# 14chanwa/remotesensingProject

Measured on AMD Instinct MI355X. Metric: Mpixel*disparity-hypotheses/s, higher is better.
Workload: dtype f32

## Files before the change

### remotesensingproject_amd/csrc/k2_reg.hpp

```cpp
#pragma once

#include "k2_scan.hpp"

namespace rslf {

#ifndef RSLF_REG_GB104
#define RSLF_REG_GB104 8
#endif
constexpr int gather_batch(int c) { return c == 1 ? 8 : 4; }
constexpr int kPadSlack = 16;

template <int SPAD, int C, bool PK, bool KONLY>
__device__ __forceinline__ void mean_shift_pass(const float (&R)[PK ? 1 : C][PK ? 1 : SPAD], const f2 (&R2)[PK ? C : 1][PK ? SPAD / 2 : 1],
                                                int S, float kq, const float (&rbar)[C], float (&A)[C], float& B)
{
    static_assert(!KONLY || (C == 1 && !PK), "the K-only pass is written for the scalar one-channel blocks");
    if constexpr (PK) {
        f2 rb2[C];
        const f2 kq2 = {kq, kq};
#pragma unroll
        for (int c = 0; c < C; c++)
            rb2[c] = f2{rbar[c], rbar[c]};
        constexpr int kBlk = (C == 1) ? 8 : 4;
#pragma unroll
        for (int s0 = 0; s0 < SPAD; s0 += kBlk) {
            if (!(s0 < SPAD - kPadSlack || s0 < S))
                continue;
            if constexpr (C == 1) {
                f2 P[4], K[4];
                const f2 r4[4] = {R2[0][s0 / 2], R2[0][s0 / 2 + 1], R2[0][s0 / 2 + 2], R2[0][s0 / 2 + 3]};
                mean_shift_pk_octet(r4, rb2[0], kq2, P, K);
#pragma unroll
                for (int j = 0; j < 4; j++) {
                    A[0] = A[0] + P[j].x;
                    B = B + K[j].x;
                    A[0] = A[0] + P[j].y;
                    B = B + K[j].y;
                }
            } else {
                f2 Pa[3], Pb[3], Ka, Kb;
                const f2 ra[3] = {R2[0][s0 / 2], R2[1][s0 / 2], R2[C - 1][s0 / 2]};
                const f2 rb[3] = {R2[0][s0 / 2 + 1], R2[1][s0 / 2 + 1], R2[C - 1][s0 / 2 + 1]};
                const f2 m[3] = {rb2[0], rb2[C > 1 ? 1 : 0], rb2[C - 1]};
                mean_shift_pk_rgb_quad(ra, rb, m, kq2, Pa, Pb, Ka, Kb);
#pragma unroll
                for (int c = 0; c < C; c++)
                    A[c] = A[c] + Pa[c].x;
                B = B + Ka.x;
#pragma unroll
                for (int c = 0; c < C; c++)
                    A[c] = A[c] + Pa[c].y;
                B = B + Ka.y;
#pragma unroll
                for (int c = 0; c < C; c++)
                    A[c] = A[c] + Pb[c].x;
                B = B + Kb.x;
#pragma unroll
                for (int c = 0; c < C; c++)
                    A[c] = A[c] + Pb[c].y;
                B = B + Kb.y;
            }
        }
    } else if (C == 1) {
#pragma unroll
        for (int s0 = 0; s0 < SPAD; s0 += 4) {
            if (s0 + 4 <= SPAD - kPadSlack || s0 + 4 <= S) {
                if constexpr (KONLY)
                    mean_shift_group4_k(R[0][s0], R[0][s0 + 1], R[0][s0 + 2], R[0][s0 + 3], rbar[0], kq, B);
                else
                    mean_shift_group4(R[0][s0], R[0][s0 + 1], R[0][s0 + 2], R[0][s0 + 3], rbar[0], kq, A[0], B);
            } else {
#pragma unroll
                for (int j = 0; j < 3; j++)
                    if (s0 + j < S) {
                        if constexpr (KONLY)
                            mean_shift_group1_k(R[0][s0 + j], rbar[0], kq, B);
                        else
                            mean_shift_group1(R[0][s0 + j], rbar[0], kq, A[0], B);
                    }
            }
        }
    } else {
#pragma unroll
        for (int s = 0; s < SPAD; s++) {
            if (!(s < SPAD - kPadSlack || s < S))
                continue;
            float q[C];
#pragma unroll
            for (int c = 0; c < C; c++) {
                const float delta = R[c][s] - rbar[c];
                const float tq = kq * delta;
                q[c] = tq * delta;
            }
            float qs = q[0];
            if (C == 3) {
                qs = q[0] + q[C - 1];
                qs = qs + q[C > 1 ? 1 : 0];
            }
            const float K = kernel_weight(qs);
#pragma unroll
            for (int c = 0; c < C; c++) {
                const float pr = R[c][s] * K;
                A[c] = A[c] + pr;
            }
            B = B + K;
        }
    }
}

template <int SPAD, int C, bool BORDER, bool UNIFORM_D, bool PK, int GB = 0, class BestT = Best<C>, bool LANE_D = false,
          bool TRIM = false>
__device__ __forceinline__ void scan_reg_body(const ScanArgs& a, int v, int u, int d0, int d1, BestT& best,
                                              float* __restrict__ otab, int dlane = 0, int dstep = 1)
{
    static_assert(!LANE_D || !UNIFORM_D, "hypotheses in the lanes: every lane has its own view offsets");
    constexpr int kGatherBatch = GB > 0 ? GB : (C == 1 && !PK && SPAD == 104 && RSLF_REG_GB104 == 13) ? 13 : gather_batch(C);
    static_assert(SPAD % kGatherBatch == 0 && (!PK || kGatherBatch % 2 == 0), "whole batches, whole pairs");
    static_assert(SPAD % 8 == 0, "slot counts are multiples of 8");
    const VolView& vol = a.vol;
    const float* epi = vol.row(v, 0);
    const float uf = (float)u;
    const int Um1 = vol.U - 1;
    const unsigned Um1_bits = __float_as_uint((float)Um1);
    const int S = vol.S;
    const int lane = threadIdx.x & 63;
    const long long o = (long long)v * vol.U + u;
    const float dmin = a.dmin_vu ? a.dmin_vu[o] : a.dmin;
    const float dmax = a.dmax_vu ? a.dmax_vu[o] : a.dmax;
    const float range = dmax - dmin;
    const float denom = (float)(a.dim_d - 1);
    const float kq = (C == 1) ? a.k.k1 : a.k.inv_h2;
    const float slope = a.k.slope;
    const int stride_s = (int)vol.stride_s;
    float centre[C];
#pragma unroll
    for (int c = 0; c < C; c++)
        centre[c] = epi[(long long)a.s_hat * vol.stride_s + u * C + c];

#pragma unroll 1
    for (int dk = d0; dk < d1; dk += (LANE_D ? dstep : 1)) {
        const int d = LANE_D ? min(dk + dlane, d1 - 1) : dk;
        const float Dd = hypothesis(dmin, range, denom, d);
        float R[PK ? 1 : C][PK ? 1 : SPAD];
        f2 R2[PK ? C : 1][PK ? SPAD / 2 : 1];
        int card = BORDER ? 0 : S;
        float Ss0 = (float)a.s_hat;
        asm volatile("" : "+v"(Ss0));
        int rowoff = 0;
        asm volatile("" : "+s"(rowoff));
        if (UNIFORM_D) {
#pragma unroll
            for (int s0 = 0; s0 < SPAD; s0 += 64) {
                const int s = s0 + lane;
                float off = (float)(a.s_hat - s) * Dd;
                off = off * slope;
                if (SPAD % 64 == 0 || s < SPAD)
                    otab[s] = off;
            }
            __builtin_amdgcn_wave_barrier();
        }
#pragma unroll
        for (int g = 0; g < SPAD / kGatherBatch; g++) {
            float tt[kGatherBatch], e0[C][kGatherBatch], e1[C][kGatherBatch];
            bool ok[kGatherBatch];
#pragma unroll
            for (int j = 0; j < kGatherBatch; j++) {
                const int s = g * kGatherBatch + j;
                tt[j] = 0.0f;
                ok[j] = false;
#pragma unroll
                for (int c = 0; c < C; c++) {
                    e0[c][j] = kSentinel;
                    e1[c][j] = 0.0f;
                }
                if (s < SPAD - kPadSlack || s < S) {
                    float x;
                    if (UNIFORM_D) {
                        x = otab[s];
                    } else {
                        x = (Ss0 - (float)s) * Dd;
                        x = x * slope;
                    }
                    x = x + uf;
                    tt[j] = lerp_weight(x);
                    int i0 = floor_to_int(x);
                    ok[j] = true;
                    if (BORDER) {
                        ok[j] = __float_as_uint(x) <= Um1_bits;
                        i0 = ok[j] ? i0 : 0;
                    }
                    const unsigned byteoff = (unsigned)(i0 * C + rowoff) << 2;
                    const float* p = (const float*)((const char*)epi + byteoff);
#pragma unroll
                    for (int c = 0; c < C; c++) {
                        e0[c][j] = p[c];
                        e1[c][j] = p[C + c];
                    }
                }
                rowoff += stride_s;
            }
#pragma unroll
            for (int j = 0; j < kGatherBatch; j++) {
                const int s = g * kGatherBatch + j;
                const float omt = 1.0f - tt[j];
#pragma unroll
                for (int c = 0; c < C; c++) {
                    const float m0 = omt * e0[c][j];
                    const float m1 = tt[j] * e1[c][j];
                    const float r = m0 + m1;
                    float val;
                    if (BORDER)
                        val = ok[j] ? r : kSentinel;
                    else
                        val = (s < SPAD - kPadSlack || s < S) ? r : kSentinel;
                    if constexpr (PK) {
                        if (s & 1)
                            R2[c][s >> 1].y = val;
                        else
                            R2[c][s >> 1].x = val;
                    } else {
                        R[c][s] = val;
                    }
                }
                if (BORDER)
                    card += ok[j] ? 1 : 0;
            }
            {
                const int b = g * kGatherBatch;
#pragma unroll
                for (int c = 0; c < C; c++) {
                    if constexpr (PK) {
                        asm volatile("" : "+v"(R2[c][b / 2]), "+v"(R2[c][b / 2 + 1]));
                        if (kGatherBatch == 8)
                            asm volatile("" : "+v"(R2[c][b / 2 + 2]), "+v"(R2[c][b / 2 + 3]));
                        static_assert(!PK || kGatherBatch == 4 || kGatherBatch == 8, "pair pinning is written for 4 and 8");
                    } else if (kGatherBatch != 4 && kGatherBatch != 8) {
#pragma unroll
                        for (int j = 0; j < kGatherBatch; j++)
                            asm volatile("" : "+v"(R[c][b + j]));
                    } else {
                        asm volatile("" : "+v"(R[c][b + 0]), "+v"(R[c][b + 1]), "+v"(R[c][b + 2]), "+v"(R[c][b + 3]));
                        if (kGatherBatch == 8)
                            asm volatile("" : "+v"(R[c][b + kGatherBatch - 4]), "+v"(R[c][b + kGatherBatch - 3]),
                                              "+v"(R[c][b + kGatherBatch - 2]), "+v"(R[c][b + kGatherBatch - 1]));
                    }
                }
                if (BORDER)
                    asm volatile("" : "+s"(rowoff), "+v"(Ss0), "+v"(card));
                else
                    asm volatile("" : "+s"(rowoff), "+v"(Ss0));
            }
        }

        float rbar[C];
#pragma unroll
        for (int c = 0; c < C; c++)
            rbar[c] = centre[c];
        float B = 0.0f;
#pragma unroll 1
        for (int it = 0; it < a.k.n_iter; it++) {
            float A[C];
#pragma unroll
            for (int c = 0; c < C; c++)
                A[c] = 0.0f;
            B = 0.0f;
            if constexpr (TRIM) {
                if (it == a.k.n_iter - 1) {
                    mean_shift_pass<SPAD, C, PK, true>(R, R2, S, kq, rbar, A, B);
                    break;
                }
            }
            mean_shift_pass<SPAD, C, PK, false>(R, R2, S, kq, rbar, A, B);
#pragma unroll
            for (int c = 0; c < C; c++) {
                const float qd = (B != 0.0f) ? (A[c] / B) : 0.0f;
                rbar[c] = (qd > 0.0f) ? qd : 0.0f;
            }
        }
        const float cardf = (float)card;
        float sc = (card != 0) ? (B / cardf) : 0.0f;
        sc = (sc > 0.0f) ? sc : 0.0f;
        if (!LANE_D || dk + dlane < d1)
            best.offer(sc, d, Dd, rbar);
    }
}

template <int C>
struct LastPassRbar {
    __device__ __forceinline__ void operator()(const ScanArgs& a, long long o, float Dd, float (&rbar)[C]) const
    {
        if (a.k.n_iter == 0)
            return;
        const VolView& vol = a.vol;
        const int v = (int)(o / vol.U);
        const int u = (int)(o - (long long)v * vol.U);
        const float* epi = vol.row(v, 0);
        const float uf = (float)u;
        const unsigned Um1_bits = __float_as_uint((float)(vol.U - 1));
        const float kq = (C == 1) ? a.k.k1 : a.k.inv_h2;
        const float Ss0 = (float)a.s_hat;
        const int S = vol.S;
        float A[C];
#pragma unroll
        for (int c = 0; c < C; c++)
            A[c] = 0.0f;
        float B = 0.0f;
        constexpr int kBatch = 8;
#pragma unroll 1
        for (int s0 = 0; s0 < S; s0 += kBatch) {
            float R[C][kBatch];
#pragma unroll
            for (int j = 0; j < kBatch; j++) {
                const int s = min(s0 + j, S - 1);
                float x = (Ss0 - (float)s) * Dd;
                x = x * a.k.slope;
                x = x + uf;
                const float t = lerp_weight(x);
                const bool ok = __float_as_uint(x) <= Um1_bits;
                const int i0 = ok ? floor_to_int(x) : 0;
                const float* p = epi + (long long)s * vol.stride_s + i0 * C;
                const float omt = 1.0f - t;
#pragma unroll
                for (int c = 0; c < C; c++) {
                    const float m0 = omt * p[c];
                    const float m1 = t * p[C + c];
                    const float r = m0 + m1;
                    R[c][j] = ok ? r : kSentinel;
                }
            }
#pragma unroll
            for (int j = 0; j < kBatch; j++) {
                if (s0 + j >= S)
                    break;
                float q[C];
#pragma unroll
                for (int c = 0; c < C; c++) {
                    const float delta = R[c][j] - rbar[c];
                    const float tq = kq * delta;
                    q[c] = tq * delta;
                }
                float qs = q[0];
                if (C == 3) {
                    qs = q[0] + q[C - 1];
                    qs = qs + q[C > 1 ? 1 : 0];
                }
                const float K = kernel_weight(qs);
#pragma unroll
                for (int c = 0; c < C; c++) {
                    const float pr = R[c][j] * K;
                    A[c] = A[c] + pr;
                }
                B = B + K;
            }
        }
#pragma unroll
        for (int c = 0; c < C; c++) {
            const float qd = (B != 0.0f) ? (A[c] / B) : 0.0f;
            rbar[c] = (qd > 0.0f) ? qd : 0.0f;
        }
    }
};

constexpr int scan_reg_waves(int spad, int c)
{
    const int regs = ((c * spad + (c == 1 ? 64 : 96) + 7) / 8) * 8;
    const int w = 512 / regs;
    if (c == 1 && spad > 104 && spad <= 144) return 3;
    if (c == 1 && spad >= 80 && spad <= 88) return 4;
    if (c == 3 && spad >= 32 && spad <= 40) return 3;
    if (c == 1 && (spad == 48 || spad == 40)) return 5;
    if (c == 3 && spad == 24) return 4;
    if (c == 1 && spad == 16) return 7;
    return w > 8 ? 8 : (w < 1 ? 1 : w);
}

#ifndef RSLF_REG_BEST_LDS
#define RSLF_REG_BEST_LDS 1
#endif
constexpr bool scan_reg_best_in_lds(int spad, int c)
{
    if (!RSLF_REG_BEST_LDS)
        return false;
    if (c == 1)
        return spad == 16 || spad == 40 || spad == 48 || (spad >= 80 && spad <= 88) || (spad >= 104 && spad <= 144);
    return spad == 24 || spad == 40;
}

constexpr bool scan_reg_packed_math(int spad, int c) { return scan_reg_waves(spad, c) == 1; }

constexpr bool scan_reg_trim(int spad, int c)
{
    return c == 1 && !scan_reg_packed_math(spad, c) && spad != 48 && !(spad >= 80 && spad <= 88) && !(spad > 112 && spad <= 144);
}
template <int SPAD, int C>
using ScanRegRbarFix = std::conditional_t<scan_reg_trim(SPAD, C), LastPassRbar<C>, NoRbarFix>;

template <int SPAD, int C, class BestT>
__device__ __forceinline__ void scan_reg_rows(const ScanArgs& a, int v, int u, int d0, int d1, BestT& best, float* otab)
{
    constexpr bool PK = scan_reg_packed_math(SPAD, C);
    if (a.dmin_vu) {
        scan_reg_body<SPAD, C, true, false, PK, 0, BestT, false, scan_reg_trim(SPAD, C)>(a, v, u, d0, d1, best, otab);
        return;
    }
    const float max_ds = (float)max(a.s_hat, a.vol.S - 1 - a.s_hat);
    const float range = a.dmax - a.dmin, denom = (float)(a.dim_d - 1);
    const float uf = (float)u, Um1 = (float)(a.vol.U - 1);
    auto interior = [&](int d) -> bool {
        const float reach = max_ds * fabsf(hypothesis(a.dmin, range, denom, d)) * fabsf(a.k.slope) + 2.0f;
        return __all((uf - reach >= 0.0f) && (uf + reach <= Um1));
    };
    int d = d0;
    while (d < d1) {
        const bool in = interior(d);
        int e = d + 1;
        while (e < d1 && interior(e) == in)
            e++;
        if (in)
            scan_reg_body<SPAD, C, false, true, PK, 0, BestT, false, scan_reg_trim(SPAD, C)>(a, v, u, d, e, best, otab);
        else
            scan_reg_body<SPAD, C, true, true, PK, 0, BestT, false, scan_reg_trim(SPAD, C)>(a, v, u, d, e, best, otab);
        d = e;
    }
}

template <int SPAD, int C>
__global__ __launch_bounds__(64 * kScanWaves) __attribute__((amdgpu_waves_per_eu(scan_reg_waves(SPAD, C), scan_reg_waves(SPAD, C))))
void k2_scan_reg(ScanArgs a)
{
    __shared__ float s_otab[kScanWaves][SPAD];
    float* otab = s_otab[__builtin_amdgcn_readfirstlane(threadIdx.x >> 6)];
    constexpr bool kEpiDyn = false;
    float* const epi_lds = nullptr;
    const int epi_stride = 0;
    using Fix = ScanRegRbarFix<SPAD, C>;
    if constexpr (scan_reg_best_in_lds(SPAD, C)) {
        __shared__ float s_best[kScanWaves][BestLds<C>::kFloats];
        BestLds<C> running(s_best[__builtin_amdgcn_readfirstlane(threadIdx.x >> 6)]);
        RSLF_SCAN_ROW_TILE_FIX((running.init(), scan_reg_rows<SPAD, C>(a, v, u, d0, d1, running, otab), running.load(best)), Fix{})
    } else {
        RSLF_SCAN_ROW_TILE_FIX((scan_reg_rows<SPAD, C>(a, v, u, d0, d1, best, otab)), Fix{})
    }
}

#ifndef RSLF_PACKED_LONG_GB
#define RSLF_PACKED_LONG_GB 4
#endif
constexpr bool packed_long_unit(int spad, int c) { return c == 1 && spad >= 80 && spad <= 128 && spad % RSLF_PACKED_LONG_GB == 0; }
constexpr int packed_waves(int spad, int c) { return packed_long_unit(spad, c) ? 2 : scan_reg_waves(spad + 24, c); }
constexpr int packed_gather_batch(int spad, int c) { return packed_long_unit(spad, c) ? spad / RSLF_PACKED_LONG_GB : 0; }

template <int SPAD, int C>
__global__ __launch_bounds__(64 * kScanWaves) __attribute__((amdgpu_waves_per_eu(packed_waves(SPAD, C), packed_waves(SPAD, C))))
void k2_scan_reg_packed(ScanArgs a)
{
    constexpr bool kEpiDyn = false;
    float* const epi_lds = nullptr;
    const int epi_stride = 0;
    RSLF_SCAN_PACKED_LOOP((scan_reg_body<SPAD, C, true, false, packed_waves(SPAD, C) == 1, packed_gather_batch(SPAD, C)>(a, v, u, d0, d1, best, nullptr)))
}

#ifndef RSLF_PX_ROWLIKE
#define RSLF_PX_ROWLIKE 1
#endif
constexpr int px_kernel_waves(int spad, int c) { return RSLF_PX_ROWLIKE ? scan_reg_waves(spad, c) : packed_waves(spad, c); }
template <int SPAD, int C>
__global__ __launch_bounds__(64 * kScanWaves) __attribute__((amdgpu_waves_per_eu(px_kernel_waves(SPAD, C), px_kernel_waves(SPAD, C))))
void k2_scan_reg_px(ScanArgs a)
{
    __shared__ double s_sum[kScanWaves];
    __shared__ float s_rec[kScanWaves][kPxRecFloats];
    const int n = *a.packed_n;
    const int lane = threadIdx.x & 63;
    const int wave = __builtin_amdgcn_readfirstlane(threadIdx.x >> 6);
    const int wpp = a.px_waves, ppw = kScanWaves / wpp;
    const int items = (n + ppw - 1) / ppw;
    const int sub = wave % wpp;
    const int dlane = sub * 64 + lane, dstep = 64 * wpp;
    for (int item = blockIdx.x; item < items; item += gridDim.x) {
        const int e = item * ppw + wave / wpp;
        const bool listed = e < n;
        const unsigned o = (unsigned)__builtin_amdgcn_readfirstlane(a.list[listed ? e : n - 1]);
        const int v = (int)(o / (unsigned)a.vol.U);
        const int u = (int)(o - (unsigned)v * (unsigned)a.vol.U);
        const bool have = listed && scan_px_owns(a, v);
        Best<C> best;
        best.init();
        const float dlo = a.dmin_vu ? a.dmin_vu[o] : a.dmin, dhi = a.dmax_vu ? a.dmax_vu[o] : a.dmax;
        const float reach = (float)max(a.s_hat, a.vol.S - 1 - a.s_hat) * fmaxf(fabsf(dlo), fabsf(dhi)) * fabsf(a.k.slope) + 2.0f;
        const bool interior = (float)u - reach >= 0.0f && (float)u + reach <= (float)(a.vol.U - 1);
        constexpr int kGB = RSLF_PX_ROWLIKE ? 0 : packed_gather_batch(SPAD, C);
        if (!have) {
        } else if (interior)
            scan_reg_body<SPAD, C, false, false, false, kGB, Best<C>, true>(a, v, u, 0, a.dim_d, best, nullptr, dlane, dstep);
        else
            scan_reg_body<SPAD, C, true, false, false, kGB, Best<C>, true>(a, v, u, 0, a.dim_d, best, nullptr, dlane, dstep);
        scan_px_finish<C>(a, o, have, best, wave, lane, wpp, s_rec, s_sum);
    }
}

}
```

### remotesensingproject_amd/csrc/rslf_device.hpp

```cpp
#pragma once

#include <hip/hip_runtime.h>
#include <stdint.h>

namespace rslf {

constexpr int kWave = 64;
constexpr float kSentinel = 1.0e30f;

struct VolView {
    const float* base;
    int V, S, U, C;
    int pitch;
    long long stride_s;
    long long stride_v;
    __device__ __forceinline__ const float* row(int v, int s) const
    {
        return base + (long long)v * stride_v + (long long)s * stride_s;
    }
};

struct ScanConsts {
    float slope;
    float inv_h2;
    float k1;
    float raw_thr;
    int   n_iter;
    int   interp;
};

struct EdgeConsts {
    int   filter_size;
    int   cut_shadows;
    float shadow_level;
    float edge_thr;
};

__device__ __forceinline__ float norm1(float x)
{
    return (float)((double)fabsf(x) * 1.73205080757);
}
__device__ __forceinline__ float norm3(float x, float y, float z)
{
    double s = (double)x * (double)x;
    s += (double)y * (double)y;
    s += (double)z * (double)z;
    return (float)sqrt(s);
}

__device__ __forceinline__ float kernel_weight(float q)
{
    float k;
    asm("v_sub_f32_e64 %0, 1.0, %1 clamp" : "=v"(k) : "v"(q));
    return k;
}

__device__ __forceinline__ float lerp_weight(float x)
{
    return __builtin_amdgcn_fractf(x);
}
__device__ __forceinline__ int floor_to_int(float x)
{
    int i;
    asm("v_cvt_flr_i32_f32_e32 %0, %1" : "=v"(i) : "v"(x));
    return i;
}

typedef float f2 __attribute__((ext_vector_type(2)));

__device__ __forceinline__ f2 kernel_weight_pk(f2 q)
{
    f2 k;
    const f2 one = {1.0f, 1.0f};
    asm("v_pk_add_f32 %0, %1, %2 neg_lo:[0,1] neg_hi:[0,1] clamp" : "=v"(k) : "v"(one), "v"(q));
    return k;
}

__device__ __forceinline__ void mean_shift_pk_octet(const f2 (&r)[4], f2 rb, f2 kq, f2 (&P)[4], f2 (&K)[4])
{
    const f2 one = {1.0f, 1.0f};
    f2 t0, t1, t2, t3;
    asm("v_pk_add_f32 %[k0], %[r0], %[rb] neg_lo:[0,1] neg_hi:[0,1]\n\t"
        "v_pk_add_f32 %[k1], %[r1], %[rb] neg_lo:[0,1] neg_hi:[0,1]\n\t"
        "v_pk_add_f32 %[k2], %[r2], %[rb] neg_lo:[0,1] neg_hi:[0,1]\n\t"
        "v_pk_add_f32 %[k3], %[r3], %[rb] neg_lo:[0,1] neg_hi:[0,1]\n\t"
        "v_pk_mul_f32 %[t0], %[kq], %[k0]\n\t"
        "v_pk_mul_f32 %[t1], %[kq], %[k1]\n\t"
        "v_pk_mul_f32 %[t2], %[kq], %[k2]\n\t"
        "v_pk_mul_f32 %[t3], %[kq], %[k3]\n\t"
        "v_pk_mul_f32 %[k0], %[k0], %[t0]\n\t"
        "v_pk_mul_f32 %[k1], %[k1], %[t1]\n\t"
        "v_pk_mul_f32 %[k2], %[k2], %[t2]\n\t"
        "v_pk_mul_f32 %[k3], %[k3], %[t3]\n\t"
        "v_pk_add_f32 %[k0], %[one], %[k0] neg_lo:[0,1] neg_hi:[0,1] clamp\n\t"
        "v_pk_add_f32 %[k1], %[one], %[k1] neg_lo:[0,1] neg_hi:[0,1] clamp\n\t"
        "v_pk_add_f32 %[k2], %[one], %[k2] neg_lo:[0,1] neg_hi:[0,1] clamp\n\t"
        "v_pk_add_f32 %[k3], %[one], %[k3] neg_lo:[0,1] neg_hi:[0,1] clamp\n\t"
        "v_pk_mul_f32 %[t0], %[r0], %[k0]\n\t"
        "v_pk_mul_f32 %[t1], %[r1], %[k1]\n\t"
        "v_pk_mul_f32 %[t2], %[r2], %[k2]\n\t"
        "v_pk_mul_f32 %[t3], %[r3], %[k3]"
        : [k0] "=&v"(K[0]), [k1] "=&v"(K[1]), [k2] "=&v"(K[2]), [k3] "=&v"(K[3]),
          [t0] "=&v"(t0), [t1] "=&v"(t1), [t2] "=&v"(t2), [t3] "=&v"(t3)
        : [r0] "v"(r[0]), [r1] "v"(r[1]), [r2] "v"(r[2]), [r3] "v"(r[3]), [rb] "v"(rb), [kq] "v"(kq), [one] "v"(one));
    P[0] = t0;
    P[1] = t1;
    P[2] = t2;
    P[3] = t3;
}

__device__ __forceinline__ void mean_shift_pk_rgb_quad(const f2 (&ra)[3], const f2 (&rb)[3], const f2 (&rbar)[3], f2 kq,
                                                       f2 (&Pa)[3], f2 (&Pb)[3], f2& Ka, f2& Kb)
{
    const f2 one = {1.0f, 1.0f};
    f2 da0, da1, da2, db0, db1, db2, ta0, ta1, ta2, tb0, tb1, tb2;
    asm("v_pk_add_f32 %[da0], %[ra0], %[m0] neg_lo:[0,1] neg_hi:[0,1]\n\t"
        "v_pk_add_f32 %[da1], %[ra1], %[m1] neg_lo:[0,1] neg_hi:[0,1]\n\t"
        "v_pk_add_f32 %[da2], %[ra2], %[m2] neg_lo:[0,1] neg_hi:[0,1]\n\t"
        "v_pk_add_f32 %[db0], %[rb0], %[m0] neg_lo:[0,1] neg_hi:[0,1]\n\t"
        "v_pk_add_f32 %[db1], %[rb1], %[m1] neg_lo:[0,1] neg_hi:[0,1]\n\t"
        "v_pk_add_f32 %[db2], %[rb2], %[m2] neg_lo:[0,1] neg_hi:[0,1]\n\t"
        "v_pk_mul_f32 %[ta0], %[kq], %[da0]\n\t"
        "v_pk_mul_f32 %[ta1], %[kq], %[da1]\n\t"
        "v_pk_mul_f32 %[ta2], %[kq], %[da2]\n\t"
        "v_pk_mul_f32 %[tb0], %[kq], %[db0]\n\t"
        "v_pk_mul_f32 %[tb1], %[kq], %[db1]\n\t"
        "v_pk_mul_f32 %[tb2], %[kq], %[db2]\n\t"
        "v_pk_mul_f32 %[da0], %[da0], %[ta0]\n\t"
        "v_pk_mul_f32 %[da2], %[da2], %[ta2]\n\t"
        "v_pk_mul_f32 %[db0], %[db0], %[tb0]\n\t"
        "v_pk_mul_f32 %[db2], %[db2], %[tb2]\n\t"
        "v_pk_mul_f32 %[da1], %[da1], %[ta1]\n\t"
        "v_pk_mul_f32 %[db1], %[db1], %[tb1]\n\t"
        "v_pk_add_f32 %[da0], %[da0], %[da2]\n\t"
        "v_pk_add_f32 %[db0], %[db0], %[db2]\n\t"
        "v_pk_add_f32 %[da0], %[da0], %[da1]\n\t"
        "v_pk_add_f32 %[db0], %[db0], %[db1]\n\t"
        "v_pk_add_f32 %[ka], %[one], %[da0] neg_lo:[0,1] neg_hi:[0,1] clamp\n\t"
        "v_pk_add_f32 %[kb], %[one], %[db0] neg_lo:[0,1] neg_hi:[0,1] clamp\n\t"
        "v_pk_mul_f32 %[ta0], %[ra0], %[ka]\n\t"
        "v_pk_mul_f32 %[ta1], %[ra1], %[ka]\n\t"
        "v_pk_mul_f32 %[ta2], %[ra2], %[ka]\n\t"
        "v_pk_mul_f32 %[tb0], %[rb0], %[kb]\n\t"
        "v_pk_mul_f32 %[tb1], %[rb1], %[kb]\n\t"
        "v_pk_mul_f32 %[tb2], %[rb2], %[kb]"
        : [da0] "=&v"(da0), [da1] "=&v"(da1), [da2] "=&v"(da2), [db0] "=&v"(db0), [db1] "=&v"(db1), [db2] "=&v"(db2),
          [ta0] "=&v"(ta0), [ta1] "=&v"(ta1), [ta2] "=&v"(ta2), [tb0] "=&v"(tb0), [tb1] "=&v"(tb1), [tb2] "=&v"(tb2),
          [ka] "=&v"(Ka), [kb] "=&v"(Kb)
        : [ra0] "v"(ra[0]), [ra1] "v"(ra[1]), [ra2] "v"(ra[2]), [rb0] "v"(rb[0]), [rb1] "v"(rb[1]), [rb2] "v"(rb[2]),
          [m0] "v"(rbar[0]), [m1] "v"(rbar[1]), [m2] "v"(rbar[2]), [kq] "v"(kq), [one] "v"(one));
    Pa[0] = ta0;
    Pa[1] = ta1;
    Pa[2] = ta2;
    Pb[0] = tb0;
    Pb[1] = tb1;
    Pb[2] = tb2;
}

__device__ __forceinline__ void mean_shift_group4(float r0, float r1, float r2, float r3, float rbar, float k1,
                                                  float& A, float& B)
{
    float t0, t1, t2, t3, u0, u1, u2, u3;
    asm("v_sub_f32 %2, %10, %14\n\t"
        "v_sub_f32 %3, %11, %14\n\t"
        "v_sub_f32 %4, %12, %14\n\t"
        "v_sub_f32 %5, %13, %14\n\t"
        "v_mul_f32 %6, %15, %2\n\t"
        "v_mul_f32 %7, %15, %3\n\t"
        "v_mul_f32 %8, %15, %4\n\t"
        "v_mul_f32 %9, %15, %5\n\t"
        "v_mul_f32 %2, %2, %6\n\t"
        "v_mul_f32 %3, %3, %7\n\t"
        "v_mul_f32 %4, %4, %8\n\t"
        "v_mul_f32 %5, %5, %9\n\t"
        "v_sub_f32_e64 %2, 1.0, %2 clamp\n\t"
        "v_sub_f32_e64 %3, 1.0, %3 clamp\n\t"
        "v_sub_f32_e64 %4, 1.0, %4 clamp\n\t"
        "v_sub_f32_e64 %5, 1.0, %5 clamp\n\t"
        "v_mul_f32 %6, %10, %2\n\t"
        "v_mul_f32 %7, %11, %3\n\t"
        "v_mul_f32 %8, %12, %4\n\t"
        "v_mul_f32 %9, %13, %5\n\t"
        "v_add_f32 %0, %0, %6\n\t"
        "v_add_f32 %1, %1, %2\n\t"
        "v_add_f32 %0, %0, %7\n\t"
        "v_add_f32 %1, %1, %3\n\t"
        "v_add_f32 %0, %0, %8\n\t"
        "v_add_f32 %1, %1, %4\n\t"
        "v_add_f32 %0, %0, %9\n\t"
        "v_add_f32 %1, %1, %5"
        : "+v"(A), "+v"(B), "=&v"(t0), "=&v"(t1), "=&v"(t2), "=&v"(t3), "=&v"(u0), "=&v"(u1), "=&v"(u2), "=&v"(u3)
        : "v"(r0), "v"(r1), "v"(r2), "v"(r3), "v"(rbar), "s"(k1));
}

__device__ __forceinline__ void mean_shift_group1(float r0, float rbar, float k1, float& A, float& B)
{
    float t0, u0;
    asm("v_sub_f32 %2, %4, %5\n\t"
        "v_mul_f32 %3, %6, %2\n\t"
        "v_mul_f32 %2, %2, %3\n\t"
        "v_sub_f32_e64 %2, 1.0, %2 clamp\n\t"
        "v_mul_f32 %3, %4, %2\n\t"
        "v_add_f32 %0, %0, %3\n\t"
        "v_add_f32 %1, %1, %2"
        : "+v"(A), "+v"(B), "=&v"(t0), "=&v"(u0)
        : "v"(r0), "v"(rbar), "s"(k1));
}

__device__ __forceinline__ void mean_shift_group4_k(float r0, float r1, float r2, float r3, float rbar, float k1, float& B)
{
    float t0, t1, t2, t3, u0, u1, u2, u3;
    asm("v_sub_f32 %1, %9, %13\n\t"
        "v_sub_f32 %2, %10, %13\n\t"
        "v_sub_f32 %3, %11, %13\n\t"
        "v_sub_f32 %4, %12, %13\n\t"
        "v_mul_f32 %5, %14, %1\n\t"
        "v_mul_f32 %6, %14, %2\n\t"
        "v_mul_f32 %7, %14, %3\n\t"
        "v_mul_f32 %8, %14, %4\n\t"
        "v_mul_f32 %1, %1, %5\n\t"
        "v_mul_f32 %2, %2, %6\n\t"
        "v_mul_f32 %3, %3, %7\n\t"
        "v_mul_f32 %4, %4, %8\n\t"
        "v_sub_f32_e64 %1, 1.0, %1 clamp\n\t"
        "v_sub_f32_e64 %2, 1.0, %2 clamp\n\t"
        "v_add_f32 %0, %0, %1\n\t"
        "v_sub_f32_e64 %3, 1.0, %3 clamp\n\t"
        "v_add_f32 %0, %0, %2\n\t"
        "v_sub_f32_e64 %4, 1.0, %4 clamp\n\t"
        "v_add_f32 %0, %0, %3\n\t"
        "v_add_f32 %0, %0, %4"
        : "+v"(B), "=&v"(t0), "=&v"(t1), "=&v"(t2), "=&v"(t3), "=&v"(u0), "=&v"(u1), "=&v"(u2), "=&v"(u3)
        : "v"(r0), "v"(r1), "v"(r2), "v"(r3), "v"(rbar), "s"(k1));
}

__device__ __forceinline__ void mean_shift_group1_k(float r0, float rbar, float k1, float& B)
{
    float t0, u0;
    asm("v_sub_f32 %1, %3, %4\n\t"
        "v_mul_f32 %2, %5, %1\n\t"
        "v_mul_f32 %1, %1, %2\n\t"
        "v_sub_f32_e64 %1, 1.0, %1 clamp\n\t"
        "v_add_f32 %0, %0, %1"
        : "+v"(B), "=&v"(t0), "=&v"(u0)
        : "v"(r0), "v"(rbar), "s"(k1));
}

__device__ __forceinline__ int reflect101(int p, int len)
{
    if (len == 1)
        return 0;
    while (p < 0 || p >= len)
        p = (p < 0) ? -p : 2 * len - 2 - p;
    return p;
}

__device__ __forceinline__ int xcd_logical_block(int b, int per_xcd)
{
    return (b & 7) * per_xcd + (b >> 3);
}

__device__ __forceinline__ int xcd_logical_block_rows(int b, int row_blocks)
{
    const int slot = b >> 3;
    const int k = slot / row_blocks;
    return ((b & 7) + 8 * k) * row_blocks + (slot - k * row_blocks);
}

}
```

Baseline: 8066.

## Precompute per-slot gather offsets and lerp weights in LDS for lane-uniform taps

When the wave covers consecutive pixels and the fractional lerp weight of a view slot is identical across all lanes, the per-slot integer offset, border limit and weight are computed once per slot into LDS tables. The gather loop then uses a simple u-relative address and shared weights instead of the per-lane floor, fract and border test. Slots where the weight differs across lanes fall back to the original path, chosen per batch through a ballot mask. This cuts per-lane VALU address arithmetic but enlarges the shared table four to fivefold, adds LDS reads per slot, and adds a branch per gather batch.

```diff
diff --git a/remotesensingproject_amd/csrc/k2_reg.hpp b/remotesensingproject_amd/csrc/k2_reg.hpp
--- a/remotesensingproject_amd/csrc/k2_reg.hpp
+++ b/remotesensingproject_amd/csrc/k2_reg.hpp
@@ -8,6 +8,7 @@
 #define RSLF_REG_GB104 8
 #endif
 constexpr int gather_batch(int c) { return c == 1 ? 8 : 4; }
+constexpr bool reg_table_pairs(int spad, int c) { return c == 1 && (spad == 96 || spad == 104); }
 constexpr int kPadSlack = 16;
 
 template <int SPAD, int C, bool PK, bool KONLY>
@@ -111,7 +112,7 @@
 template <int SPAD, int C, bool BORDER, bool UNIFORM_D, bool PK, int GB = 0, class BestT = Best<C>, bool LANE_D = false,
           bool TRIM = false>
 __device__ __forceinline__ void scan_reg_body(const ScanArgs& a, int v, int u, int d0, int d1, BestT& best,
-                                              float* __restrict__ otab, int dlane = 0, int dstep = 1)
+                                              float* __restrict__ otab, int dlane = 0, int dstep = 1, int span = -1)
 {
     static_assert(!LANE_D || !UNIFORM_D, "hypotheses in the lanes: every lane has its own view offsets");
     constexpr int kGatherBatch = GB > 0 ? GB : (C == 1 && !PK && SPAD == 104 && RSLF_REG_GB104 == 13) ? 13 : gather_batch(C);
@@ -136,6 +137,12 @@
 #pragma unroll
     for (int c = 0; c < C; c++)
         centre[c] = epi[(long long)a.s_hat * vol.stride_s + u * C + c];
+    constexpr bool kPairs = reg_table_pairs(SPAD, C);
+    constexpr int kWords = (SPAD + 63) / 64;
+    const int u0 = UNIFORM_D ? __builtin_amdgcn_readfirstlane(u) : 0;
+    int* const tab_off = reinterpret_cast<int*>(otab + SPAD);
+    int* const tab_lim = reinterpret_cast<int*>(otab + 2 * SPAD);
+    float* const tab_t = otab + 3 * SPAD;
 
 #pragma unroll 1
     for (int dk = d0; dk < d1; dk += (LANE_D ? dstep : 1)) {
@@ -148,83 +155,154 @@
         asm volatile("" : "+v"(Ss0));
         int rowoff = 0;
         asm volatile("" : "+s"(rowoff));
+        unsigned long long mixed[kWords];
         if (UNIFORM_D) {
+            int ln = lane, tu0 = u0;
+            asm volatile("" : "+v"(ln), "+s"(tu0));
 #pragma unroll
             for (int s0 = 0; s0 < SPAD; s0 += 64) {
-                const int s = s0 + lane;
+                const int s = s0 + ln;
                 float off = (float)(a.s_hat - s) * Dd;
                 off = off * slope;
-                if (SPAD % 64 == 0 || s < SPAD)
+                const UniformTap ut = uniform_tap(off, tu0, span);
+                if (SPAD % 64 == 0 || s < SPAD) {
                     otab[s] = off;
+                    tab_off[s] = ((ut.i0 - tu0) * C + s * stride_s) << 2;
+                    tab_lim[s] = tu0 + Um1 - ut.i0 - (ut.t != 0.0f ? 1 : 0);
+                    if (kPairs)
+                        reinterpret_cast<f2*>(tab_t)[s] = f2{ut.t, 1.0f - ut.t};
+                    else
+                        tab_t[s] = ut.t;
+                }
+                mixed[s0 / 64] = __ballot(s < S && !ut.uniform);
             }
             __builtin_amdgcn_wave_barrier();
         }
 #pragma unroll
         for (int g = 0; g < SPAD / kGatherBatch; g++) {
-            float tt[kGatherBatch], e0[C][kGatherBatch], e1[C][kGatherBatch];
-            bool ok[kGatherBatch];
-#pragma unroll
-            for (int j = 0; j < kGatherBatch; j++) {
-                const int s = g * kGatherBatch + j;
-                tt[j] = 0.0f;
-                ok[j] = false;
-#pragma unroll
-                for (int c = 0; c < C; c++) {
-                    e0[c][j] = kSentinel;
-                    e1[c][j] = 0.0f;
-                }
-                if (s < SPAD - kPadSlack || s < S) {
-                    float x;
-                    if (UNIFORM_D) {
-                        x = otab[s];
-                    } else {
-                        x = (Ss0 - (float)s) * Dd;
-                        x = x * slope;
-                    }
-                    x = x + uf;
-                    tt[j] = lerp_weight(x);
-                    int i0 = floor_to_int(x);
-                    ok[j] = true;
-                    if (BORDER) {
-                        ok[j] = __float_as_uint(x) <= Um1_bits;
-                        i0 = ok[j] ? i0 : 0;
-                    }
-                    const unsigned byteoff = (unsigned)(i0 * C + rowoff) << 2;
-                    const float* p = (const float*)((const char*)epi + byteoff);
+            if (UNIFORM_D && !any_slot(mixed, g * kGatherBatch, kGatherBatch)) {
+                float e0[C][kGatherBatch], e1[C][kGatherBatch];
+                bool ok[kGatherBatch];
+#pragma unroll
+                for (int j = 0; j < kGatherBatch; j++) {
+                    const int s = g * kGatherBatch + j;
+                    ok[j] = false;
 #pragma unroll
                     for (int c = 0; c < C; c++) {
-                        e0[c][j] = p[c];
-                        e1[c][j] = p[C + c];
-                    }
-                }
-                rowoff += stride_s;
-            }
-#pragma unroll
-            for (int j = 0; j < kGatherBatch; j++) {
-                const int s = g * kGatherBatch + j;
-                const float omt = 1.0f - tt[j];
-#pragma unroll
-                for (int c = 0; c < C; c++) {
-                    const float m0 = omt * e0[c][j];
-                    const float m1 = tt[j] * e1[c][j];
-                    const float r = m0 + m1;
-                    float val;
+                        e0[c][j] = kSentinel;
+                        e1[c][j] = 0.0f;
+                    }
+                    if (s < SPAD - kPadSlack || s < S) {
+                        int up = u;
+                        ok[j] = true;
+                        if (BORDER) {
+                            const int lim = tab_lim[s];
+                            ok[j] = u <= lim;
+                            up = min(u, lim);
+                        }
+                        const unsigned byteoff = (unsigned)(up * (C * 4) + tab_off[s]);
+                        const float* p = (const float*)((const char*)epi + byteoff);
+#pragma unroll
+                        for (int c = 0; c < C; c++) {
+                            e0[c][j] = p[c];
+                            e1[c][j] = p[C + c];
+                        }
+                    }
+                }
+#pragma unroll
+                for (int j = 0; j < kGatherBatch; j++) {
+                    const int s = g * kGatherBatch + j;
+                    const f2 w = kPairs ? reinterpret_cast<const f2*>(tab_t)[s] : f2{tab_t[s], 0.0f};
+                    const float t = w.x;
+                    const float omt = kPairs ? w.y : 1.0f - t;
+#pragma unroll
+                    for (int c = 0; c < C; c++) {
+                        const float m0 = omt * e0[c][j];
+                        const float m1 = t * e1[c][j];
+                        const float r = m0 + m1;
+                        const float val = (BORDER ? ok[j] : (s < SPAD - kPadSlack || s < S)) ? r : kSentinel;
+                        if constexpr (PK) {
+                            if (s & 1)
+                                R2[c][s >> 1].y = val;
+                            else
+                                R2[c][s >> 1].x = val;
+                        } else {
+                            R[c][s] = val;
+                        }
+                    }
                     if (BORDER)
-                        val = ok[j] ? r : kSentinel;
-                    else
-                        val = (s < SPAD - kPadSlack || s < S) ? r : kSentinel;
-                    if constexpr (PK) {
-                        if (s & 1)
-                            R2[c][s >> 1].y = val;
+                        card += ok[j] ? 1 : 0;
+                }
+            } else {
+                int ro_copy = rowoff;
+                int& ro = UNIFORM_D ? ro_copy : rowoff;
+                float tt[kGatherBatch], e0[C][kGatherBatch], e1[C][kGatherBatch];
+                bool ok[kGatherBatch];
+#pragma unroll
+                for (int j = 0; j < kGatherBatch; j++) {
+                    const int s = g * kGatherBatch + j;
+                    tt[j] = 0.0f;
+                    ok[j] = false;
+#pragma unroll
+                    for (int c = 0; c < C; c++) {
+                        e0[c][j] = kSentinel;
+                        e1[c][j] = 0.0f;
+                    }
+                    if (s < SPAD - kPadSlack || s < S) {
+                        float x;
+                        if (UNIFORM_D) {
+                            x = otab[s];
+                        } else {
+                            x = (Ss0 - (float)s) * Dd;
+                            x = x * slope;
+                        }
+                        x = x + uf;
+                        tt[j] = lerp_weight(x);
+                        int i0 = floor_to_int(x);
+                        ok[j] = true;
+                        if (BORDER) {
+                            ok[j] = __float_as_uint(x) <= Um1_bits;
+                            i0 = ok[j] ? i0 : 0;
+                        }
+                        const unsigned byteoff = (unsigned)(i0 * C + ro) << 2;
+                        const float* p = (const float*)((const char*)epi + byteoff);
+#pragma unroll
+                        for (int c = 0; c < C; c++) {
+                            e0[c][j] = p[c];
+                            e1[c][j] = p[C + c];
+                        }
+                    }
+                    ro += stride_s;
+                }
+#pragma unroll
+                for (int j = 0; j < kGatherBatch; j++) {
+                    const int s = g * kGatherBatch + j;
+                    const float omt = 1.0f - tt[j];
+#pragma unroll
+                    for (int c = 0; c < C; c++) {
+                        const float m0 = omt * e0[c][j];
+                        const float m1 = tt[j] * e1[c][j];
+                        const float r = m0 + m1;
+                        float val;
+                        if (BORDER)
+                            val = ok[j] ? r : kSentinel;
                         else
-                            R2[c][s >> 1].x = val;
-                    } else {
-                        R[c][s] = val;
-                    }
-                }
-                if (BORDER)
-                    card += ok[j] ? 1 : 0;
-            }
+                            val = (s < SPAD - kPadSlack || s < S) ? r : kSentinel;
+                        if constexpr (PK) {
+                            if (s & 1)
+                                R2[c][s >> 1].y = val;
+                            else
+                                R2[c][s >> 1].x = val;
+                        } else {
+                            R[c][s] = val;
+                        }
+                    }
+                    if (BORDER)
+                        card += ok[j] ? 1 : 0;
+                }
+            }
+            if (UNIFORM_D)
+                rowoff += kGatherBatch * stride_s;
             {
                 const int b = g * kGatherBatch;
 #pragma unroll
@@ -395,6 +473,8 @@
 template <int SPAD, int C>
 using ScanRegRbarFix = std::conditional_t<scan_reg_trim(SPAD, C), LastPassRbar<C>, NoRbarFix>;
 
+constexpr int reg_table_floats(int spad, int c) { return (reg_table_pairs(spad, c) ? 5 : 4) * spad; }
+
 template <int SPAD, int C, class BestT>
 __device__ __forceinline__ void scan_reg_rows(const ScanArgs& a, int v, int u, int d0, int d1, BestT& best, float* otab)
 {
@@ -406,6 +486,10 @@
     const float max_ds = (float)max(a.s_hat, a.vol.S - 1 - a.s_hat);
     const float range = a.dmax - a.dmin, denom = (float)(a.dim_d - 1);
     const float uf = (float)u, Um1 = (float)(a.vol.U - 1);
+    const int lane = threadIdx.x & 63;
+    const int u0 = __builtin_amdgcn_readfirstlane(u);
+    const int last = __builtin_amdgcn_readlane(u, 63);
+    const int span = __all(u == u0 + min(lane, last - u0)) ? last - u0 : -1;
     auto interior = [&](int d) -> bool {
         const float reach = max_ds * fabsf(hypothesis(a.dmin, range, denom, d)) * fabsf(a.k.slope) + 2.0f;
         return __all((uf - reach >= 0.0f) && (uf + reach <= Um1));
@@ -417,9 +501,9 @@
         while (e < d1 && interior(e) == in)
             e++;
         if (in)
-            scan_reg_body<SPAD, C, false, true, PK, 0, BestT, false, scan_reg_trim(SPAD, C)>(a, v, u, d, e, best, otab);
+            scan_reg_body<SPAD, C, false, true, PK, 0, BestT, false, scan_reg_trim(SPAD, C)>(a, v, u, d, e, best, otab, 0, 1, span);
         else
-            scan_reg_body<SPAD, C, true, true, PK, 0, BestT, false, scan_reg_trim(SPAD, C)>(a, v, u, d, e, best, otab);
+            scan_reg_body<SPAD, C, true, true, PK, 0, BestT, false, scan_reg_trim(SPAD, C)>(a, v, u, d, e, best, otab, 0, 1, span);
         d = e;
     }
 }
@@ -428,7 +512,7 @@
 __global__ __launch_bounds__(64 * kScanWaves) __attribute__((amdgpu_waves_per_eu(scan_reg_waves(SPAD, C), scan_reg_waves(SPAD, C))))
 void k2_scan_reg(ScanArgs a)
 {
-    __shared__ float s_otab[kScanWaves][SPAD];
+    __shared__ __attribute__((aligned(16))) float s_otab[kScanWaves][reg_table_floats(SPAD, C)];
     float* otab = s_otab[__builtin_amdgcn_readfirstlane(threadIdx.x >> 6)];
     constexpr bool kEpiDyn = false;
     float* const epi_lds = nullptr;
diff --git a/remotesensingproject_amd/csrc/rslf_device.hpp b/remotesensingproject_amd/csrc/rslf_device.hpp
--- a/remotesensingproject_amd/csrc/rslf_device.hpp
+++ b/remotesensingproject_amd/csrc/rslf_device.hpp
@@ -64,6 +64,35 @@
     int i;
     asm("v_cvt_flr_i32_f32_e32 %0, %1" : "=v"(i) : "v"(x));
     return i;
+}
+
+struct UniformTap {
+    bool uniform;
+    int i0;
+    float t;
+};
+__device__ __forceinline__ UniformTap uniform_tap(float off, int u0, int span)
+{
+    const float x0 = off + (float)u0;
+    const float x1 = off + (float)(u0 + span);
+    UniformTap r;
+    r.i0 = floor_to_int(x0);
+    r.t = lerp_weight(x0);
+    r.uniform = span >= 0 && x0 >= 0.0f && floor_to_int(x1) - r.i0 == span && lerp_weight(x1) == r.t;
+    return r;
+}
+
+template <int W>
+__device__ __forceinline__ bool any_slot(const unsigned long long (&m)[W], int b, int n)
+{
+    bool any = false;
+#pragma unroll
+    for (int w = 0; w < W; w++) {
+        const int lo = max(b - 64 * w, 0), hi = min(b + n - 64 * w, 64);
+        if (lo < hi)
+            any = any || ((m[w] >> lo) & (hi - lo == 64 ? ~0ull : (1ull << (hi - lo)) - 1)) != 0;
+    }
+    return any;
 }
 
 typedef float f2 __attribute__((ext_vector_type(2)));
```

Result: faster. 8178, median of 6 (+1.4%).
